# gh2o/CS184-Raytracer

Measured on NVIDIA B200. Metric: Mrays/s (primary+shadow+secondary), higher is better.
Workload: dtype f64

## Files before the change

cs184-raytracer_b200/csrc/rt_device.cuh:

```cuda
#pragma once
#include <cuda_runtime.h>
#include <stdint.h>

#include "rt_b200.h"

namespace rt {

struct d3 {
    double x, y, z;
};

__device__ __forceinline__ d3 mk3(double x, double y, double z) { d3 r; r.x = x; r.y = y; r.z = z; return r; }
__device__ __forceinline__ d3 operator+(d3 a, d3 b) { return mk3(a.x + b.x, a.y + b.y, a.z + b.z); }
__device__ __forceinline__ d3 operator-(d3 a, d3 b) { return mk3(a.x - b.x, a.y - b.y, a.z - b.z); }
__device__ __forceinline__ d3 operator-(d3 a) { return mk3(-a.x, -a.y, -a.z); }
__device__ __forceinline__ d3 operator*(double s, d3 a) { return mk3(s * a.x, s * a.y, s * a.z); }
__device__ __forceinline__ d3 vdiv(d3 a, double s) { return mk3(a.x / s, a.y / s, a.z / s); }

__device__ __forceinline__ double sum4(double a, double b, double c, double d) { return (a + c) + (b + d); }
__device__ __forceinline__ double dot4(d3 a, d3 b) { return sum4(a.x * b.x, a.y * b.y, a.z * b.z, 0.0); }
__device__ __forceinline__ double norm4(d3 a) { return sqrt(dot4(a, a)); }
__device__ __forceinline__ d3 ray_normalize(d3 a) { return vdiv(a, norm4(a)); }
__device__ __forceinline__ d3 inplace_normalize(d3 a) { return (1.0 / norm4(a)) * a; }

__device__ __forceinline__ d3 xf_point(const double* __restrict__ m, d3 v) {
    return mk3(((m[0] * v.x + m[1] * v.y) + m[2] * v.z) + m[3] * 1.0,
               ((m[4] * v.x + m[5] * v.y) + m[6] * v.z) + m[7] * 1.0,
               ((m[8] * v.x + m[9] * v.y) + m[10] * v.z) + m[11] * 1.0);
}
__device__ __forceinline__ d3 xf_dir(const double* __restrict__ m, d3 v) {
    return mk3(((m[0] * v.x + m[1] * v.y) + m[2] * v.z) + m[3] * 0.0,
               ((m[4] * v.x + m[5] * v.y) + m[6] * v.z) + m[7] * 0.0,
               ((m[8] * v.x + m[9] * v.y) + m[10] * v.z) + m[11] * 0.0);
}
__device__ __forceinline__ d3 xf_normal(const double* __restrict__ inv, d3 n) {
    return mk3(sum4(inv[0] * n.x, inv[4] * n.y, inv[8] * n.z, 0.0),
               sum4(inv[1] * n.x, inv[5] * n.y, inv[9] * n.z, 0.0),
               sum4(inv[2] * n.x, inv[6] * n.y, inv[10] * n.z, 0.0));
}

__device__ __forceinline__ double det3(d3 c0, d3 c1, d3 c2) {
    double h012 = c0.x * (c1.y * c2.z - c2.y * c1.z);
    double h102 = c1.x * (c0.y * c2.z - c2.y * c0.z);
    double h201 = c2.x * (c0.y * c1.z - c1.y * c0.z);
    return h012 - h102 + h201;
}

struct alignas(16) DGeom {
    double inv[12];
    double fwd[12];
    double det;
    double center[3];
    double radius2;
    double bbmin[3];
    double bbmax[3];
    int type;
    int mat;
    int first_face;
    int num_faces;
    int use_bbox;
    int pad_[3];
};

struct alignas(16) DMat {
    double ka[3], kd[3], ks[3], kr[3];
    double sp, ior;
    int has_kt;
    int has_kr;
    int pad_[2];
};

struct alignas(16) DLight {
    double v[3];
    double color[3];
    double falloff;
    int type;
    int pad_;
};

struct DCamera {
    double eye[3], ll[3], lr[3], ul[3], ur[3];
};

#define RT_FACE_D2 5

struct alignas(128) BvhNode {
    float4 lox, loy, loz;
    int4 ref;
    float4 hix, hiy, hiz;
    int4 pad_;
};
#define BVH_EMPTY_LO 1e30f
#define BVH_EMPTY_HI (-1e30f)
#define BVH_DONE ((int)0x80000000)

#define PRIM_KIND_SHIFT 29
#define PRIM_FACE 0
#define PRIM_SPHERE 1
#define PRIM_TRI 2
#define PRIM_INDEX_MASK ((1 << PRIM_KIND_SHIFT) - 1)

struct DScene {
    DCamera cam;
    const DGeom* geoms;
    const DMat* mats;
    const DLight* slights;
    const DLight* alights;
    const double2* face_pts;
    const double2* face_nrm;
    const BvhNode* nodes;
    const int* flat;
    const int* all_prims;
    const float4* sph_bound;
    int num_geoms;
    int num_slights;
    int num_alights;
    int num_flat;
    int num_all;
    int num_bvh_prims;
    int single_leaf;
    int shadow_mode;
    float origin_limit;
};

struct Best {
    int geom;
    int face;
    double dobj;
    double wd;
    d3 P, N;
};

struct ObjRay {
    int geom;
    int box_ok;
    d3 o, d, nd;
    double dn;
};

struct WorkCounters {
    unsigned long long nodes, tris, spheres;
};

__device__ __forceinline__ bool bbox_plane(const double* oo, const double* dd, int axis, int bn, const double* __restrict__ bbmin,
                                           const double* __restrict__ bbmax) {
    const double mag = dd[axis];
    if (mag == 0.0) return false;
    const double t = ((bn ? bbmax[axis] : bbmin[axis]) - oo[axis]) / mag;
    if (t < 0) return false;
    bool ok = true;
#pragma unroll
    for (int a2 = 0; a2 < 3; a2++) {
        if (a2 == axis) continue;
        const double ip = oo[a2] + t * dd[a2];
        if (ip < bbmin[a2] || ip > bbmax[a2]) ok = false;
    }
    return ok;
}
__device__ __forceinline__ bool mesh_bbox(d3 o, d3 d, const double* __restrict__ bbmin,
                                          const double* __restrict__ bbmax) {
    const double oo[3] = {o.x, o.y, o.z}, dd[3] = {d.x, d.y, d.z};
    {
        float best = 3.0e38f;
        int baxis = 0, bbn = 0;
#pragma unroll
        for (int axis = 0; axis < 3; axis++) {
            const float df = (float)dd[axis];
            if (df == 0.f) continue;
            const int bn = df > 0.f ? 1 : 0;
            const float tf = ((float)(bn ? bbmax[axis] : bbmin[axis]) - (float)oo[axis]) / df;
            if (tf >= 0.f && tf < best) { best = tf; baxis = axis; bbn = bn; }
        }
        if (best < 3.0e38f) {
            bool hit;
            if (baxis == 0) hit = bbox_plane(oo, dd, 0, bbn, bbmin, bbmax);
            else if (baxis == 1) hit = bbox_plane(oo, dd, 1, bbn, bbmin, bbmax);
            else hit = bbox_plane(oo, dd, 2, bbn, bbmin, bbmax);
            if (hit) return true;
        }
    }
#pragma unroll
    for (int axis = 0; axis < 3; axis++) {
#pragma unroll
        for (int bn = 0; bn < 2; bn++)
            if (bbox_plane(oo, dd, axis, bn, bbmin, bbmax)) return true;
    }
    return false;
}

__device__ __forceinline__ void load_objray(const DScene& S, int gi, d3 o, d3 d, ObjRay& R) {
    const DGeom* g = S.geoms + gi;
    R.geom = gi;
    R.o = xf_point(g->inv, o);
    R.d = ray_normalize(xf_dir(g->inv, d));
    R.nd = -R.d;
    R.dn = sqrt(R.d.x * R.d.x + (R.d.y * R.d.y + R.d.z * R.d.z));
    R.box_ok = 1;
    if (g->type == RT_GEOM_MESH && g->use_bbox) R.box_ok = mesh_bbox(R.o, R.d, g->bbmin, g->bbmax) ? 1 : 0;
}

__device__ __forceinline__ bool beats(const Best& best, int gi, int f, double dobj, double wd) {
    if (best.geom < 0) return true;
    if (gi == best.geom) return dobj < best.dobj || (dobj == best.dobj && f < best.face);
    return wd < best.wd || (wd == best.wd && gi < best.geom);
}

__device__ __forceinline__ void to_world(const DGeom* g, d3 Pobj, d3 Nobj, d3 o, d3& P, d3& N, double& wd) {
    P = xf_point(g->fwd, Pobj);
    N = xf_normal(g->inv, Nobj);
    if (g->det < 0) N = -N;
    wd = norm4(P - o);
}

template <bool ANYHIT>
__device__ __forceinline__ bool test_sphere(const DScene& S, int gi, d3 o, d3 d, bool reverse, double limit,
                                            Best& best) {
    const DGeom* g = S.geoms + gi;
    d3 oo = xf_point(g->inv, o);
    d3 dd = ray_normalize(xf_dir(g->inv, d));
    d3 c = mk3(g->center[0], g->center[1], g->center[2]);
    d3 ocd = oo - c;
    double a = dot4(dd, dd);
    double b = 2 * dot4(dd, ocd);
    double cc = dot4(ocd, ocd) - g->radius2;
    double disc = b * b - 4 * a * cc;
    if (disc < 0) return false;
    double res = reverse ? (-b + sqrt(disc)) / (2 * a) : (-b - sqrt(disc)) / (2 * a);
    if (res < 0) return false;
    d3 Pobj = oo + res * dd;
    d3 Nobj = Pobj - c;
    d3 P, N;
    double wd;
    to_world(g, Pobj, Nobj, o, P, N, wd);
    if (ANYHIT) return wd <= limit;
    if (beats(best, gi, 0, 0.0, wd)) {
        best.geom = gi; best.face = 0; best.dobj = 0.0; best.wd = wd; best.P = P; best.N = N;
    }
    return false;
}

template <bool ANYHIT>
__device__ __forceinline__ bool test_face(const DScene& S, int gi, int gface, int lface, const ObjRay& R, d3 o,
                                          bool reverse, double limit, Best& best) {
    const double2* __restrict__ fp = S.face_pts + (size_t)gface * RT_FACE_D2;
    double2 q0 = __ldg(fp + 0), q1 = __ldg(fp + 1), q2 = __ldg(fp + 2), q3 = __ldg(fp + 3), q4 = __ldg(fp + 4);
    d3 p0 = mk3(q0.x, q0.y, q1.x), va = mk3(q1.y, q2.x, q2.y), vb = mk3(q3.x, q3.y, q4.x);
    d3 rhs = R.o - p0;
    double dlower = det3(va, vb, R.nd);
    if (dlower == 0) return false;
    double a = det3(rhs, vb, R.nd) / dlower;
    if (a < 0 || a > 1) return false;
    double b = det3(va, rhs, R.nd) / dlower;
    if (b < 0 || a + b > 1) return false;
    double t = det3(va, vb, rhs) / dlower;
    if (t < 0) return false;
    double dobj = t * R.dn;
    if (!ANYHIT && best.geom == gi && (dobj > best.dobj || (dobj == best.dobj && lface > best.face))) return false;
    const double2* __restrict__ fn = S.face_nrm + (size_t)gface * RT_FACE_D2;
    double2 m0 = __ldg(fn + 0), m1 = __ldg(fn + 1), m2 = __ldg(fn + 2), m3 = __ldg(fn + 3), m4 = __ldg(fn + 4);
    d3 n0 = mk3(m0.x, m0.y, m1.x), n1 = mk3(m1.y, m2.x, m2.y), n2 = mk3(m3.x, m3.y, m4.x);
    double w0 = 1.0 - a - b;
    d3 tn = (w0 * n0 + a * n1) + b * n2;
    bool front = dot4(tn, R.d) < 0;
    if ((!front) != reverse) return false;
    d3 Pobj = p0 + (a * va + b * vb);
    d3 P, N;
    double wd;
    to_world(S.geoms + gi, Pobj, tn, o, P, N, wd);
    if (ANYHIT) return wd <= limit;
    if (beats(best, gi, lface, dobj, wd)) {
        best.geom = gi; best.face = lface; best.dobj = dobj; best.wd = wd; best.P = P; best.N = N;
    }
    return false;
}

__device__ __forceinline__ bool sphere_certainly_missed(float4 bs, d3 o, d3 d) {
    float ocx = bs.x - (float)o.x, ocy = bs.y - (float)o.y, ocz = bs.z - (float)o.z;
    float dx = (float)d.x, dy = (float)d.y, dz = (float)d.z;
    float c2 = ocx * ocx + ocy * ocy + ocz * ocz;
    float b = ocx * dx + ocy * dy + ocz * dz;
    float r = bs.w * 1.001f;
    float r2 = r * r + 1e-4f * c2 + 1e-30f;
    if (c2 - b * b > r2) return true;
    return c2 > r2 && b < -(r + 1e-3f * sqrtf(c2));
}

template <bool ANYHIT, bool COUNT>
__device__ __forceinline__ bool test_prim(const DScene& S, int code, d3 o, d3 d, bool reverse, double limit,
                                          ObjRay& R, Best& best, WorkCounters& wc) {
    const int kind = code >> PRIM_KIND_SHIFT, idx = code & PRIM_INDEX_MASK;
    if (kind == PRIM_SPHERE) {
        if (sphere_certainly_missed(__ldg(S.sph_bound + idx), o, d)) return false;
        if (COUNT) wc.spheres++;
        return test_sphere<ANYHIT>(S, idx, o, d, reverse, limit, best);
    }
    if (kind == PRIM_TRI) {
        const DGeom* g = S.geoms + idx;
        if (R.geom != idx) load_objray(S, idx, o, d, R);
        if (COUNT) wc.tris += 2;
        if (test_face<ANYHIT>(S, idx, g->first_face, 0, R, o, reverse, limit, best)) return true;
        return test_face<ANYHIT>(S, idx, g->first_face + 1, 1, R, o, reverse, limit, best);
    }
    double2 q4 = __ldg(S.face_pts + (size_t)idx * RT_FACE_D2 + 4);
    int gi = __double2loint(q4.y), lf = __double2hiint(q4.y);
    if (R.geom != gi) load_objray(S, gi, o, d, R);
    if (!R.box_ok) return false;
    if (COUNT) wc.tris++;
    return test_face<ANYHIT>(S, gi, idx, lf, R, o, reverse, limit, best);
}

struct FRay {
    float ix, iy, iz;
    float bx, by, bz;
    unsigned nx, ny, nz;
};
__device__ __forceinline__ FRay make_fray(d3 o, d3 d) {
    FRay r;
    float ox = (float)o.x, oy = (float)o.y, oz = (float)o.z;
    float dx = (float)d.x, dy = (float)d.y, dz = (float)d.z;
    const float tiny = 1e-30f;
    if (fabsf(dx) < tiny) dx = copysignf(tiny, dx);
    if (fabsf(dy) < tiny) dy = copysignf(tiny, dy);
    if (fabsf(dz) < tiny) dz = copysignf(tiny, dz);
    r.ix = 1.0f / dx; r.iy = 1.0f / dy; r.iz = 1.0f / dz;
    r.bx = -ox * r.ix; r.by = -oy * r.iy; r.bz = -oz * r.iz;
    r.nx = r.ix < 0.f ? 64u : 0u;
    r.ny = r.iy < 0.f ? 80u : 16u;
    r.nz = r.iz < 0.f ? 96u : 32u;
    asm volatile("" : "+r"(r.nx), "+r"(r.ny), "+r"(r.nz));
    return r;
}
struct Slab4 {
    float tn[4];
    bool hit[4];
};
__device__ __forceinline__ void slab1(const FRay& r, float nx, float ny, float nz, float fx, float fy, float fz,
                                      float tlimit, float& tn, bool& hit) {
    const float tnx = __fmaf_rn(nx, r.ix, r.bx), tny = __fmaf_rn(ny, r.iy, r.by), tnz = __fmaf_rn(nz, r.iz, r.bz);
    const float tfx = __fmaf_rn(fx, r.ix, r.bx), tfy = __fmaf_rn(fy, r.iy, r.by), tfz = __fmaf_rn(fz, r.iz, r.bz);
    tn = fmaxf(fmaxf(tnx, tny), fmaxf(tnz, 0.f));
    const float tf = fminf(fminf(tfx, tfy), fminf(tfz, tlimit));
    hit = tn <= tf;
}

#define RT_STACK 96
#ifndef RT_ANYHIT_UNSORTED
#define RT_ANYHIT_UNSORTED 1
#endif
#ifndef RT_SH_STACK
#define RT_SH_STACK 12
#endif
#ifndef RT_BLOCK
#define RT_BLOCK 64
#endif

__device__ __forceinline__ float prune_limit(double x) {
    if (!(x < 3.0e38)) return __int_as_float(0x7f800000);
    return __double2float_ru(x) * 1.00001f + 1e-30f;
}

#define RT_SH_ENTRY(ANYHIT) ((ANYHIT) ? 4 : 8)
#define RT_SH_STRIDE(ANYHIT) (RT_BLOCK * RT_SH_ENTRY(ANYHIT))
#define RT_SH_STACK_BYTES(ANYHIT) ((RT_SH_STACK > 0 ? RT_SH_STACK : 1) * RT_SH_STRIDE(ANYHIT))

template <bool ANYHIT>
__device__ __forceinline__ unsigned stack_base(const void* smem) {
    unsigned b = (unsigned)__cvta_generic_to_shared(smem) + threadIdx.x * RT_SH_ENTRY(ANYHIT);
    asm volatile("" : "+r"(b));
    return b;
}

template <bool ANYHIT>
struct StackSpill {
    int ref[RT_STACK];
    float t[ANYHIT ? 1 : RT_STACK];
};
template <bool ANYHIT>
struct Stack {
    unsigned base, top;
    StackSpill<ANYHIT>& sp;
    __device__ __forceinline__ Stack(unsigned shbase, StackSpill<ANYHIT>& spill) : base(shbase), top(shbase), sp(spill) {}
    __device__ __forceinline__ unsigned lim() const { return base + RT_SH_STACK * RT_SH_STRIDE(ANYHIT); }
    __device__ __forceinline__ static void sts(unsigned a, int ref, float t) {
        if (ANYHIT) asm volatile("st.shared.b32 [%0], %1;" ::"r"(a), "r"(ref));
        else asm volatile("st.shared.v2.b32 [%0], {%1, %2};" ::"r"(a), "r"(ref), "r"(__float_as_int(t)));
    }
    __device__ __forceinline__ bool roomy(int n) const { return top + n * RT_SH_STRIDE(ANYHIT) <= lim(); }
    __device__ __forceinline__ void push_fast(bool on, int ref, float t) {
        if (on) sts(top, ref, t);
        top += on ? RT_SH_STRIDE(ANYHIT) : 0;
    }
    __device__ __forceinline__ void push(int ref, float t) {
        if (top < lim()) {
            sts(top, ref, t);
        } else {
            const unsigned k = (top - lim()) / RT_SH_STRIDE(ANYHIT);
            if (k >= RT_STACK) return;
            sp.ref[k] = ref;
            if (!ANYHIT) sp.t[k] = t;
        }
        top += RT_SH_STRIDE(ANYHIT);
    }
    __device__ __forceinline__ int pop(float tlim) {
        while (top != base) {
            top -= RT_SH_STRIDE(ANYHIT);
            int ref, tb = 0;
            if (top < lim()) {
                if (ANYHIT) asm volatile("ld.shared.b32 %0, [%1];" : "=r"(ref) : "r"(top));
                else asm volatile("ld.shared.v2.b32 {%0, %1}, [%2];" : "=r"(ref), "=r"(tb) : "r"(top));
            } else {
                const unsigned k = (top - lim()) / RT_SH_STRIDE(ANYHIT);
                ref = sp.ref[k];
                if (!ANYHIT) tb = __float_as_int(sp.t[k]);
            }
            if (ANYHIT || __int_as_float(tb) <= tlim) return ref;
        }
        return BVH_DONE;
    }
};

__device__ __forceinline__ const float4* flip64(const float4* p) {
    return reinterpret_cast<const float4*>(reinterpret_cast<unsigned long long>(p) ^ 64ull);
}

template <bool ANYHIT, bool COUNT>
__device__ __forceinline__ void descend(const DScene& S, const FRay& fr, float tlim, int& cur, Stack<ANYHIT>& st,
                                        WorkCounters& wc) {
    while (cur >= 0) {
        const char* const nb = reinterpret_cast<const char*>(S.nodes);
        const unsigned off = (unsigned)cur * (unsigned)sizeof(BvhNode);
        const float4* pnx = reinterpret_cast<const float4*>(nb + (off + fr.nx));
        const float4* pny = reinterpret_cast<const float4*>(nb + (off + fr.ny));
        const float4* pnz = reinterpret_cast<const float4*>(nb + (off + fr.nz));
        const float4 nx = __ldg(pnx), ny = __ldg(pny), nz = __ldg(pnz);
        const float4 fx = __ldg(flip64(pnx)), fy = __ldg(flip64(pny)), fz = __ldg(flip64(pnz));
        const int4 ref = __ldg(reinterpret_cast<const int4*>(nb + off + 48));
        if (COUNT) wc.nodes += 4;
        float t0, t1, t2, t3;
        bool h0, h1, h2, h3;
        slab1(fr, nx.x, ny.x, nz.x, fx.x, fy.x, fz.x, tlim, t0, h0);
        slab1(fr, nx.y, ny.y, nz.y, fx.y, fy.y, fz.y, tlim, t1, h1);
        slab1(fr, nx.z, ny.z, nz.z, fx.z, fy.z, fz.z, tlim, t2, h2);
        slab1(fr, nx.w, ny.w, nz.w, fx.w, fy.w, fz.w, tlim, t3, h3);
        if (ANYHIT && RT_ANYHIT_UNSORTED) {
            int next = h3 ? ref.w : BVH_DONE;
            if (st.roomy(3)) {
                bool q;
                q = h2 && next != BVH_DONE; st.push_fast(q, next, 0.f); next = h2 ? ref.z : next;
                q = h1 && next != BVH_DONE; st.push_fast(q, next, 0.f); next = h1 ? ref.y : next;
                q = h0 && next != BVH_DONE; st.push_fast(q, next, 0.f); next = h0 ? ref.x : next;
            } else {
                if (h2) { if (next != BVH_DONE) st.push(next, 0.f); next = ref.z; }
                if (h1) { if (next != BVH_DONE) st.push(next, 0.f); next = ref.y; }
                if (h0) { if (next != BVH_DONE) st.push(next, 0.f); next = ref.x; }
            }
            cur = next != BVH_DONE ? next : st.pop(tlim);
            continue;
        }
        const unsigned MISS = 0x7f800000u;
        const unsigned k0 = h0 ? ((__float_as_uint(t0) & ~3u) | 0u) : MISS, k1 = h1 ? ((__float_as_uint(t1) & ~3u) | 1u) : MISS;
        const unsigned k2 = h2 ? ((__float_as_uint(t2) & ~3u) | 2u) : MISS, k3 = h3 ? ((__float_as_uint(t3) & ~3u) | 3u) : MISS;
        const unsigned kmin = min(min(k0, k1), min(k2, k3));
        if (st.roomy(3)) {
            st.push_fast(h3 && k3 != kmin, ref.w, t3);
            st.push_fast(h2 && k2 != kmin, ref.z, t2);
            st.push_fast(h1 && k1 != kmin, ref.y, t1);
            st.push_fast(h0 && k0 != kmin, ref.x, t0);
        } else {
            if (h3 && k3 != kmin) st.push(ref.w, t3);
            if (h2 && k2 != kmin) st.push(ref.z, t2);
            if (h1 && k1 != kmin) st.push(ref.y, t1);
            if (h0 && k0 != kmin) st.push(ref.x, t0);
        }
        if (kmin < MISS) {
            const unsigned i = kmin & 3u;
            cur = i == 0 ? ref.x : (i == 1 ? ref.y : (i == 2 ? ref.z : ref.w));
        } else {
            cur = st.pop(tlim);
        }
    }
}

template <bool ANYHIT, bool BRUTE, bool COUNT, bool FARCHECK = false>
__device__ __forceinline__ bool cast_ray(const DScene& S, d3 o, d3 d, bool reverse, double limit, Best& best,
                                         WorkCounters& wc, unsigned shbase) {
    best.geom = -1; best.face = -1; best.dobj = 0.0; best.wd = 0.0;
    ObjRay R;
    R.geom = -1; R.box_ok = 1;
    const bool far_origin = FARCHECK && !BRUTE && fmax(fabs(o.x), fmax(fabs(o.y), fabs(o.z))) > (double)S.origin_limit;
    if (BRUTE || far_origin) {
        for (int i = 0; i < S.num_all; i++)
            if (test_prim<ANYHIT, COUNT>(S, __ldg(S.all_prims + i), o, d, reverse, limit, R, best, wc)) return true;
        return false;
    }
    for (int i = 0; i < S.num_flat; i++)
        if (test_prim<ANYHIT, COUNT>(S, __ldg(S.flat + i), o, d, reverse, limit, R, best, wc)) return true;
    if (S.num_bvh_prims == 0) return false;
    if (S.num_bvh_prims == 1)
        return test_prim<ANYHIT, COUNT>(S, S.single_leaf, o, d, reverse, limit, R, best, wc);

    const FRay fr = make_fray(o, d);
    float tlim = ANYHIT ? prune_limit(limit) : __int_as_float(0x7f800000);
    StackSpill<ANYHIT> spill;
    Stack<ANYHIT> st(shbase, spill);
    int cur = 0;
    while (true) {
        descend<ANYHIT, COUNT>(S, fr, tlim, cur, st, wc);
        if (cur == BVH_DONE) break;
        if (test_prim<ANYHIT, COUNT>(S, ~cur, o, d, reverse, limit, R, best, wc)) return true;
        if (!ANYHIT && best.geom >= 0) tlim = prune_limit(best.wd);
        cur = st.pop(tlim);
        if (cur == BVH_DONE) break;
    }
    return false;
}

}
```

cs184-raytracer_b200/csrc/rt_kernels.cuh:

```cuda
#pragma once
#include "rt_device.cuh"

namespace rt {

#ifndef RT_BLOCK
#define RT_BLOCK 64
#endif
#ifndef RT_SHADOW_MINBLOCKS
#define RT_SHADOW_MINBLOCKS 16
#endif
#ifndef RT_SHADOW_TILE
#define RT_SHADOW_TILE 4096
#endif
#ifndef RT_TRACE_MINBLOCKS
#define RT_TRACE_MINBLOCKS 16
#endif

struct RayQ {
    double* f;
    int* pixel;
    int* meta;
    size_t cap;
    __device__ __forceinline__ double& fld(int k, size_t i) const { return f[(size_t)k * cap + i]; }
};
// ... 31 lines not shown
    int x = (w % (RT_TILE_W / 8)) * 8 + (l & 7), y = (w / (RT_TILE_W / 8)) * 4 + (l >> 3);
    px = tx * RT_TILE_W + x;
    py = ty * RT_TILE_H + y;
    return px < F.width && py < F.height;
}

__device__ __forceinline__ unsigned warp_append(bool flag, unsigned long long* counter) {
    unsigned m = __ballot_sync(0xffffffffu, flag);
    unsigned base = 0;
    if (m) {
        int lane = threadIdx.x & 31, leader = __ffs(m) - 1;
        if (lane == leader) base = (unsigned)atomicAdd(counter, (unsigned long long)__popc(m));
        base = __shfl_sync(0xffffffffu, base, leader);
        base += __popc(m & ((1u << lane) - 1u));
    }
    return base;
}

template <bool COUNT>
__device__ __forceinline__ void flush_work(const WorkCounters& wc, unsigned long long* ctr ) {
    if (!COUNT) return;
    unsigned long long a = wc.nodes, b = wc.tris, c = wc.spheres;
    for (int o = 16; o > 0; o >>= 1) {
        a += __shfl_down_sync(0xffffffffu, a, o);
        b += __shfl_down_sync(0xffffffffu, b, o);
        c += __shfl_down_sync(0xffffffffu, c, o);
    }
    if ((threadIdx.x & 31) == 0) {
        atomicAdd(ctr + 0, a);
        atomicAdd(ctr + 1, b);
        atomicAdd(ctr + 2, c);
    }
}

struct PrimaryRays {
    FrameInfo F;
    long long first_slot;
    int sub;
    int depth;
};
__device__ __forceinline__ int primary_ray(const DScene& S, const PrimaryRays& pr, int i, d3& E, d3& d, double& w) {
    const int ss = pr.sub * pr.sub;
    const long long slot = pr.first_slot + (pr.sub > 1 ? i / ss : i);
    int px, py;
    if (!slot_to_pixel(pr.F, slot, px, py)) return -1;
    double rowFrac = (py + 0.5) / pr.F.height, colFrac = (px + 0.5) / pr.F.width;
    w = 1.0;
    if (pr.sub > 1) {
        const int k = i % ss, si = k % pr.sub, sj = k / pr.sub;
        rowFrac = (py + (sj + 0.5) / pr.sub) / pr.F.height;
        colFrac = (px + (si + 0.5) / pr.sub) / pr.F.width;
        w = 1.0 / ss;
    }
    const DCamera& c = S.cam;
    d3 LR = mk3(c.lr[0], c.lr[1], c.lr[2]), UR = mk3(c.ur[0], c.ur[1], c.ur[2]);
    d3 LL = mk3(c.ll[0], c.ll[1], c.ll[2]), UL = mk3(c.ul[0], c.ul[1], c.ul[2]);
    E = mk3(c.eye[0], c.eye[1], c.eye[2]);
    d3 right = rowFrac * LR + (1.0 - rowFrac) * UR;
    d3 left = rowFrac * LL + (1.0 - rowFrac) * UL;
    d3 ip = colFrac * right + (1.0 - colFrac) * left;
    d3 raw = ip - E;
    const bool ok = !(raw.x == 0 && raw.y == 0 && raw.z == 0);
    d = ok ? ray_normalize(raw) : raw;
    return ok ? (int)slot : -1;
}

__global__ void __launch_bounds__(RT_BLOCK) k_raygen(DScene S, PrimaryRays pr, int n, RayQ q) {
    int i = blockIdx.x * blockDim.x + threadIdx.x;
    if (i >= n) return;
    d3 E = mk3(0, 0, 0), d = mk3(0, 0, 1);
    double w = 1.0;
    const int slot = primary_ray(S, pr, i, E, d, w);
    q.fld(0, i) = E.x; q.fld(1, i) = E.y; q.fld(2, i) = E.z;
    q.fld(3, i) = d.x; q.fld(4, i) = d.y; q.fld(5, i) = d.z;
    q.fld(6, i) = w; q.fld(7, i) = w; q.fld(8, i) = w;
    q.pixel[i] = slot;
    q.meta[i] = pr.depth;
}

template <bool BRUTE, bool COUNT, bool PRIMARY>
__global__ void __launch_bounds__(RT_BLOCK, RT_TRACE_MINBLOCKS) k_trace(DScene S, RayQ q, size_t off, int n, size_t nfront, HitQ h,
                                                     unsigned long long* ctr, int* ids_geom, int* ids_face, PrimaryRays pr) {
    __shared__ __align__(16) unsigned char sm_stack[RT_SH_STACK_BYTES(false)];
    int t = blockIdx.x * blockDim.x + threadIdx.x;
    const size_t g = off + (size_t)t;
    const size_t i = PRIMARY ? 0 : (g < nfront ? g : q.cap - 1 - (g - nfront));
    bool active = t < n;
    Best best;
    best.geom = -1;
    WorkCounters wc = {0, 0, 0};
    d3 o = mk3(0, 0, 0), d = mk3(0, 0, 1);
    double w0 = 1.0;
    int meta = 0, pixel = -1;
    if (PRIMARY) {
        if (active) pixel = primary_ray(S, pr, t, o, d, w0);
        meta = pr.depth;
    } else {
        pixel = active ? q.pixel[i] : -1;
    }
    active = active && pixel >= 0;
    if (active) {
        if (!PRIMARY) {
            o = mk3(q.fld(0, i), q.fld(1, i), q.fld(2, i));
            d = mk3(q.fld(3, i), q.fld(4, i), q.fld(5, i));
            meta = q.meta[i];
        }
        cast_ray<false, BRUTE, COUNT>(S, o, d, (meta >> RT_META_INSIDE_SHIFT) & 1, 0.0, best, wc, stack_base<false>(sm_stack));
        if (ids_geom) { ids_geom[pixel] = best.geom; ids_face[pixel] = best.face; }
    }
    bool hit = active && best.geom >= 0;
    unsigned slot = warp_append(hit, ctr + CTR_HITS);
    if (hit) {
        h.fld(0, slot) = best.P.x; h.fld(1, slot) = best.P.y; h.fld(2, slot) = best.P.z;
        h.fld(3, slot) = best.N.x; h.fld(4, slot) = best.N.y; h.fld(5, slot) = best.N.z;
        h.fld(6, slot) = d.x; h.fld(7, slot) = d.y; h.fld(8, slot) = d.z;
        if (PRIMARY) { h.fld(9, slot) = w0; h.fld(10, slot) = w0; h.fld(11, slot) = w0; }
        else { h.fld(9, slot) = q.fld(6, i); h.fld(10, slot) = q.fld(7, i); h.fld(11, slot) = q.fld(8, i); }
        h.fld(12, slot) = best.wd;
        h.pixel[slot] = pixel;
        h.geom[slot] = best.geom;
        h.meta[slot] = meta;
    }
    flush_work<COUNT>(wc, ctr + CTR_NODES);
}

struct SortGrid {
    float lo[3];
    float scale;
    int bits;
};
__device__ __forceinline__ uint32_t spread_bits3(uint32_t v) {
    v = (v * 0x00010001u) & 0xFF0000FFu;
    v = (v * 0x00000101u) & 0x0F00F00Fu;
    v = (v * 0x00000011u) & 0xC30C30C3u;
    v = (v * 0x00000005u) & 0x49249249u;
    return v;
}
__global__ void k_hit_keys(HitQ h, const unsigned long long* __restrict__ lc, SortGrid g, uint32_t* __restrict__ keys,
                           int* __restrict__ vals) {
    unsigned j = blockIdx.x * blockDim.x + threadIdx.x;
    if (j >= (unsigned)lc[CTR_HITS]) return;
    const float p[3] = {(float)h.fld(0, j), (float)h.fld(1, j), (float)h.fld(2, j)};
    uint32_t q[3];
    for (int a = 0; a < 3; a++) {
        float u = (p[a] - g.lo[a]) * g.scale;
        q[a] = (uint32_t)min(max((int)u, 0), 1023);
    }
    const uint32_t m = (spread_bits3(q[0]) << 2) | (spread_bits3(q[1]) << 1) | spread_bits3(q[2]);
    keys[j] = g.bits < 30 ? m >> (30 - g.bits) : m;
    vals[j] = (int)j;
}
__global__ void __launch_bounds__(RT_BLOCK) k_shade_io(HitQ h, const unsigned long long* ctr, double* fb,
                                                        unsigned long long* maxbits) {
    unsigned j = blockIdx.x * blockDim.x + threadIdx.x;
    double v = 0.0;
    if (j < (unsigned)ctr[CTR_HITS]) {
        double dist = h.fld(12, j);
        v = 1.0 / (dist * dist);
        size_t p = (size_t)h.pixel[j] * 3;
        fb[p] = v; fb[p + 1] = v; fb[p + 2] = v;
    }
    unsigned long long b = (unsigned long long)__double_as_longlong(v);
    for (int o = 16; o > 0; o >>= 1) {
        unsigned long long x = __shfl_down_sync(0xffffffffu, b, o);
        b = x > b ? x : b;
    }
    if ((threadIdx.x & 31) == 0 && b) atomicMax(maxbits, b);
}

__global__ void k_divide(double* fb, size_t n, const unsigned long long* maxbits) {
    size_t i = (size_t)blockIdx.x * blockDim.x + threadIdx.x;
    if (i >= n) return;
    fb[i] = fb[i] / __longlong_as_double((long long)*maxbits);
}

#ifndef RT_SHADE_BLOCK
#define RT_SHADE_BLOCK 256
#endif
__global__ void __launch_bounds__(RT_SHADE_BLOCK) k_shade(DScene S, HitQ src, HitQ h, const int* __restrict__ order,
                                                     unsigned long long* ctr, RayQ next, double* fb) {
    unsigned j = blockIdx.x * blockDim.x + threadIdx.x;
    bool active = j < (unsigned)ctr[CTR_HITS];
    bool want_t = false, want_r = false;
    d3 P = mk3(0, 0, 0), Td = P, Rd = P;
    double W[3] = {0, 0, 0}, kr[3] = {0, 0, 0};
    int pixel = 0, depth = 0, inside = 0;
    unsigned degenerate = 0;
    if (active) {
        const unsigned s = order ? (unsigned)order[j] : j;
        P = mk3(src.fld(0, s), src.fld(1, s), src.fld(2, s));
        d3 N = mk3(src.fld(3, s), src.fld(4, s), src.fld(5, s));
        d3 V = mk3(src.fld(6, s), src.fld(7, s), src.fld(8, s));
        W[0] = src.fld(9, s); W[1] = src.fld(10, s); W[2] = src.fld(11, s);
        pixel = src.pixel[s];
        int meta = src.meta[s];
        const int geom = src.geom[s];
        depth = meta & RT_META_DEPTH_MASK;
// ... 57 lines not shown
        next.pixel[sr] = pixel;
        next.meta[sr] = (depth - 1) | (inside << RT_META_INSIDE_SHIFT);
    }
    if (degenerate) atomicAdd(ctr + CTR_DEGENERATE, (unsigned long long)degenerate);
}

__device__ __forceinline__ double pow_shading(double x, double y) {
    if (y >= 1.0 && y <= 1024.0 && y == floor(y)) {
        unsigned n = (unsigned)y;
        double r = 1.0, b = x;
        while (true) {
            if (n & 1u) r *= b;
            n >>= 1;
            if (!n) break;
            b *= b;
        }
        return r;
    }
    return pow(x, y);
}

template <bool BRUTE, bool COUNT>
__global__ void __launch_bounds__(RT_BLOCK, RT_SHADOW_MINBLOCKS) k_shadow(DScene S, HitQ h, unsigned long long* ctr, double* fb) {
    __shared__ __align__(16) unsigned char sm_stack[RT_SH_STACK_BYTES(true)];
    unsigned long long t = (unsigned long long)blockIdx.x * blockDim.x + threadIdx.x;
    const unsigned nsl = (unsigned)S.num_slights;
    WorkCounters wc = {0, 0, 0};
    const unsigned long long nhits = ctr[CTR_HITS];
    if (t < nhits * nsl) {
        unsigned li, j;
        if (S.shadow_mode & 1) {
#if RT_SHADOW_TILE > 0
            unsigned long long tile;
            if (nhits * nsl <= 0xffffffffull) tile = (unsigned)t / (RT_SHADOW_TILE * nsl);
            else tile = t / ((unsigned long long)RT_SHADOW_TILE * nsl);
            const unsigned long long first = tile * RT_SHADOW_TILE;
            const unsigned w = (unsigned)min((unsigned long long)RT_SHADOW_TILE, nhits - first);
            const unsigned r = (unsigned)(t - tile * RT_SHADOW_TILE * nsl);
            li = r / w; j = (unsigned)first + r % w;
#else
            li = (unsigned)(t / nhits); j = (unsigned)(t % nhits);
#endif
        } else { j = (unsigned)(t / nsl); li = (unsigned)(t % nsl); }
        const DLight* l = S.slights + li;
        d3 P = mk3(h.fld(0, j), h.fld(1, j), h.fld(2, j));
        d3 N = mk3(h.fld(3, j), h.fld(4, j), h.fld(5, j));
        d3 lv = mk3(l->v[0], l->v[1], l->v[2]);
        const bool point = l->type == RT_LIGHT_POINT;
        d3 toL = point ? lv - P : -lv;
        if (toL.x == 0 && toL.y == 0 && toL.z == 0) {
            atomicAdd(ctr + CTR_DEGENERATE, 1ull);
        } else {
            d3 L = ray_normalize(toL);
            double ndl = dot4(N, L);
            bool lrev = ndl < 0;
            const double INF = __longlong_as_double(0x7ff0000000000000ll);
            double dL = point ? norm4(toL) : INF;
            int inside = (h.meta[j] >> RT_META_INSIDE_SHIFT) & 1;
            const DMat* m = S.mats + S.geoms[h.geom[j]].mat;
            d3 V = mk3(h.fld(6, j), h.fld(7, j), h.fld(8, j));
            double att[3];
            if (point) {
                const double fo = l->falloff;
                double f = fo == 0.0 ? 1.0 : (fo == 1.0 ? 1.0 / dL : (fo == 2.0 ? 1.0 / (dL * dL) : pow(dL, -fo)));
                for (int k = 0; k < 3; k++) att[k] = f * l->color[k];
            } else {
                for (int k = 0; k < 3; k++) att[k] = l->color[k];
            }
            double di = ndl < 0.0 ? 0.0 : ndl;
            d3 R = (2 * ndl) * N - L;
            double mvr = -dot4(V, R);
            const double sp_ = m->sp;
            double si = (mvr < 0.0 && sp_ > 0.0) ? 0.0 : pow_shading(mvr < 0.0 ? 0.0 : mvr, sp_);
            double c[3];
            bool any = false;
            for (int k = 0; k < 3; k++) {
                double w = h.fld(9 + k, j);
                c[k] = w * (di * att[k] * m->kd[k]) + w * (si * att[k] * m->ks[k]);
                any = any || !(c[k] == 0.0);
            }
            if (COUNT && !any) atomicAdd(ctr + CTR_S_CULLED, 1ull);
            if (any) {
                Best best;
                bool occluded = cast_ray<true, BRUTE, COUNT>(S, P, L, lrev != (inside != 0), dL, best, wc, stack_base<true>(sm_stack));
                if (!occluded) {
                    int pixel = h.pixel[j];
                    for (int k = 0; k < 3; k++) atomicAdd(fb + (size_t)pixel * 3 + k, c[k]);
                }
            }
        }
    }
    flush_work<COUNT>(wc, ctr + CTR_S_NODES);
}

__device__ __forceinline__ unsigned char quantize(double v) {
    v = (1.0 < v) ? 1.0 : v;
    v = (v < 0.0) ? 0.0 : v;
    if (v != v) v = 0.0;
    return (unsigned char)(int)(v * 255.0);
}
template <bool QUANT>
__global__ void k_resolve(FrameInfo F, const double* __restrict__ fb, long long nslots, int full, void* out) {
    long long slot = (long long)blockIdx.x * blockDim.x + threadIdx.x;
    if (slot >= nslots) return;
    int px, py;
    bool inside = slot_to_pixel(F, slot, px, py);
    size_t dst;
    if (full) {
        if (!inside) return;
        dst = ((size_t)py * F.width + px) * 3;
    } else {
        dst = (size_t)slot * 3;
    }
    for (int k = 0; k < 3; k++) {
        double v = inside ? fb[(size_t)slot * 3 + k] : 0.0;
        if (QUANT) ((unsigned char*)out)[dst + k] = quantize(v);
        else ((double*)out)[dst + k] = v;
    }
}

#if RT_TILE_W == 32
__global__ void __launch_bounds__(256) k_resolve_rgb8_rows(FrameInfo F, const double* __restrict__ fb, long long nslots,
                                                            unsigned char* __restrict__ out) {
    __shared__ __align__(16) unsigned char rows[8][96];
    const long long slot0 = (long long)blockIdx.x * 256;
    const long long slot = slot0 + threadIdx.x;
    int px, py;
    const bool inside = slot < nslots && slot_to_pixel(F, slot, px, py);
    {
        const int j = threadIdx.x, w = j >> 5, l = j & 31;
        const int x = (w & 3) * 8 + (l & 7), y = (w >> 2) * 4 + (l >> 3);
        for (int k = 0; k < 3; k++) rows[y][3 * x + k] = inside ? quantize(fb[(size_t)slot * 3 + k]) : 0;
    }
    __syncthreads();
    int px0, py0;
    if (slot0 >= nslots) return;
    slot_to_pixel(F, slot0, px0, py0);
    if (threadIdx.x < 192) {
        const int r = threadIdx.x / 24, wd = threadIdx.x % 24;
        const int y = py0 + r;
        if (y < F.height) {
            const size_t base = ((size_t)y * F.width + px0) * 3;
            if (px0 + 32 <= F.width && (base & 3) == 0) {
                *reinterpret_cast<unsigned*>(out + base + 4 * wd) = *reinterpret_cast<const unsigned*>(&rows[r][4 * wd]);
            } else {
                const int nb = 3 * min(32, F.width - px0);
                for (int bidx = 4 * wd; bidx < 4 * wd + 4; bidx++)
                    if (bidx < nb) out[base + bidx] = rows[r][bidx];
            }
        }
    }
}
#endif

template <typename T>
__global__ void k_unpack(int width, int height, int tiles_x, int world, long long max_tiles,
                         const int* __restrict__ rank_row_start , int tiles_y,
                         const T* __restrict__ packed, T* __restrict__ frame) {
    long long i = (long long)blockIdx.x * blockDim.x + threadIdx.x;
    if (i >= (long long)width * height) return;
    int px = (int)(i % width), py = (int)(i / width);
    int tx = px / RT_TILE_W, ty = py / RT_TILE_H;
    int rank = (tx + ty) % world;
    int first_tx = ((rank - ty) % world + world) % world;
    long long lt = rank_row_start[rank * (tiles_y + 1) + ty] + (tx - first_tx) / world;
    int x = px % RT_TILE_W, y = py % RT_TILE_H;
    int w = (y / 4) * (RT_TILE_W / 8) + (x / 8), l = (y % 4) * 8 + (x % 8);
    long long slot = ((long long)rank * max_tiles + lt) * RT_TILE_PIXELS + w * 32 + l;
    for (int k = 0; k < 3; k++) frame[i * 3 + k] = packed[slot * 3 + k];
}

template <bool BRUTE>
__global__ void __launch_bounds__(RT_BLOCK) k_query(DScene S, long long n, const double* __restrict__ org,
                                                     const double* __restrict__ dir,
                                                     const unsigned char* __restrict__ reverse, int* geom, int* face,
                                                     double* dist, double* point, double* normal) {
    __shared__ __align__(16) unsigned char sm_stack[RT_SH_STACK_BYTES(false)];
    long long i = (long long)blockIdx.x * blockDim.x + threadIdx.x;
    if (i >= n) return;
    d3 o = mk3(org[3 * i], org[3 * i + 1], org[3 * i + 2]);
    d3 raw = mk3(dir[3 * i], dir[3 * i + 1], dir[3 * i + 2]);
    Best best;
    best.geom = -1; best.face = -1; best.wd = 0; best.P = mk3(0, 0, 0); best.N = mk3(0, 0, 0);
    WorkCounters wc = {0, 0, 0};
    if (raw.x == 0 && raw.y == 0 && raw.z == 0) {
        best.geom = -2;
    } else {
        cast_ray<false, BRUTE, false, true>(S, o, ray_normalize(raw), reverse ? reverse[i] != 0 : false, 0.0, best, wc, stack_base<false>(sm_stack));
    }
    bool hit = best.geom >= 0;
    if (geom) geom[i] = best.geom;
    if (face) face[i] = hit ? best.face : -1;
    if (dist) dist[i] = hit ? best.wd : 0.0;
    if (point) { point[3 * i] = hit ? best.P.x : 0; point[3 * i + 1] = hit ? best.P.y : 0; point[3 * i + 2] = hit ? best.P.z : 0; }
    if (normal) { normal[3 * i] = hit ? best.N.x : 0; normal[3 * i + 1] = hit ? best.N.y : 0; normal[3 * i + 2] = hit ? best.N.z : 0; }
}

__global__ void k_gather_probe(const float4* __restrict__ data, unsigned long long nrec, int loads, float* sink) {
    unsigned long long t = (unsigned long long)blockIdx.x * blockDim.x + threadIdx.x;
    unsigned long long x = t * 0x9E3779B97F4A7C15ull + 0x1234567ull;
    float acc = 0.f;
    for (int i = 0; i < loads; i++) {
        x ^= x >> 30; x *= 0xBF58476D1CE4E5B9ull; x ^= x >> 27; x *= 0x94D049BB133111EBull; x ^= x >> 31;
        unsigned long long r = x % nrec;
        float4 a = __ldg(data + 2 * r), b = __ldg(data + 2 * r + 1);
        acc += a.x + b.w;
    }
    if (acc == 123.456f) *sink = acc;
}

__global__ void __launch_bounds__(RT_BLOCK, RT_SHADOW_MINBLOCKS) k_node_walk(const BvhNode* __restrict__ nodes, int visits,
                                                                              int group, float* sink) {
    const unsigned t = blockIdx.x * blockDim.x + threadIdx.x;
    const unsigned path = t / (unsigned)group;
    unsigned long long x = (unsigned long long)path * 0x9E3779B97F4A7C15ull + 0x1234567ull;
    x ^= x >> 30; x *= 0xBF58476D1CE4E5B9ull; x ^= x >> 27;
    const unsigned nx = (x & 1) ? 64u : 0u, ny = (x & 2) ? 80u : 16u, nz = (x & 4) ? 96u : 32u;
    float acc = 0.f;
    int cur = 0;
    const char* const nb = reinterpret_cast<const char*>(nodes);
    for (int v = 0; v < visits; v++) {
        const unsigned off = (unsigned)cur * (unsigned)sizeof(BvhNode);
        const float4* pnx = reinterpret_cast<const float4*>(nb + (off + nx));
        const float4* pny = reinterpret_cast<const float4*>(nb + (off + ny));
        const float4* pnz = reinterpret_cast<const float4*>(nb + (off + nz));
        const float4 a = __ldg(pnx), b = __ldg(pny), c = __ldg(pnz);
        const float4 d = __ldg(flip64(pnx)), e = __ldg(flip64(pny)), f = __ldg(flip64(pnz));
        const int4 ref = __ldg(reinterpret_cast<const int4*>(nb + off + 48));
        acc += a.x + b.y + c.z + d.w + e.x + f.y;
        x = x * 6364136223846793005ull + 1442695040888963407ull;
        const unsigned r = (unsigned)(x >> 33);
        const int cand[4] = {ref.x, ref.y, ref.z, ref.w};
        int next = 0;
#pragma unroll
        for (int k = 3; k >= 0; k--) {
            const int cc = cand[(r + k) & 3];
            next = cc >= 0 ? cc : next;
        }
        cur = next;
    }
    if (acc == 123.456f) *sink = acc;
}

struct FaceOwner {
    int geom, first, count;
    int all_off;
    int bvh_off;
};

__global__ void k_pack_faces(long long nf, const double* __restrict__ pts, const double* __restrict__ nrm,
                             const FaceOwner* __restrict__ owners, int nowners, double2* __restrict__ out_p,
                             double2* __restrict__ out_n, int* __restrict__ all_prims, int* __restrict__ bvh_prims) {
    long long f = (long long)blockIdx.x * blockDim.x + threadIdx.x;
    if (f >= nf) return;
    int lo = 0, hi = nowners;
    while (lo < hi) {
        int mid = (lo + hi) >> 1;
        if (owners[mid].first <= (int)f) lo = mid + 1;
        else hi = mid;
    }
    int fgeom = 0, flocal = 0;
    if (lo > 0) {
        const FaceOwner o = owners[lo - 1];
        if ((int)f - o.first < o.count) {
            fgeom = o.geom;
            flocal = (int)f - o.first;
            if (o.all_off >= 0) {
                const int code = (PRIM_FACE << PRIM_KIND_SHIFT) | (int)f;
                all_prims[o.all_off + flocal] = code;
                bvh_prims[o.bvh_off + flocal] = code;
            }
        }
    }
    const double* p = pts + 9 * f;
    const double* n = nrm + 9 * f;
    d3 p0 = mk3(p[0], p[1], p[2]), p1 = mk3(p[3], p[4], p[5]), p2 = mk3(p[6], p[7], p[8]);
    d3 va = p1 - p0, vb = p2 - p0;
    double aux = __hiloint2double(flocal, fgeom);
// ... 21 lines not shown
```

Before: 4885.

## Spill ray/objray state to shared memory and recompute hit surface after traversal

Drops the hit point and normal from the per-thread best-hit record and recomputes them once after traversal by re-intersecting the winning primitive. In the trace and query kernels, the world and object-space ray (origin, direction, norm) now live in a per-thread shared-memory slot read through inline PTX, and the shadow kernel keeps them in a register array. It also removes the cached negated direction and skips faces early when the cached object-ray bbox test failed. The aim is to cut register pressure in the hot traversal loop and raise occupancy, at the cost of extra shared loads per primitive test and a second intersection per hit.

```diff
diff --git a/cs184-raytracer_b200/csrc/rt_device.cuh b/cs184-raytracer_b200/csrc/rt_device.cuh
--- a/cs184-raytracer_b200/csrc/rt_device.cuh
+++ b/cs184-raytracer_b200/csrc/rt_device.cuh
@@ -5,6 +5,10 @@
 #include "rt_b200.h"
 
 namespace rt {
+
+#ifndef RT_BLOCK
+#define RT_BLOCK 64
+#endif
 
 struct d3 {
     double x, y, z;
@@ -128,13 +132,12 @@
     int face;
     double dobj;
     double wd;
-    d3 P, N;
 };
 
 struct ObjRay {
     int geom;
     int box_ok;
-    d3 o, d, nd;
+    d3 o, d;
     double dn;
 };
 
@@ -193,7 +196,6 @@
     R.geom = gi;
     R.o = xf_point(g->inv, o);
     R.d = ray_normalize(xf_dir(g->inv, d));
-    R.nd = -R.d;
     R.dn = sqrt(R.d.x * R.d.x + (R.d.y * R.d.y + R.d.z * R.d.z));
     R.box_ok = 1;
     if (g->type == RT_GEOM_MESH && g->use_bbox) R.box_ok = mesh_bbox(R.o, R.d, g->bbmin, g->bbmax) ? 1 : 0;
@@ -212,10 +214,7 @@
     wd = norm4(P - o);
 }
 
-template <bool ANYHIT>
-__device__ __forceinline__ bool test_sphere(const DScene& S, int gi, d3 o, d3 d, bool reverse, double limit,
-                                            Best& best) {
-    const DGeom* g = S.geoms + gi;
+__device__ __forceinline__ bool sphere_hit(const DGeom* g, d3 o, d3 d, bool reverse, d3& P, d3& N, double& wd) {
     d3 oo = xf_point(g->inv, o);
     d3 dd = ray_normalize(xf_dir(g->inv, d));
     d3 c = mk3(g->center[0], g->center[1], g->center[2]);
@@ -229,33 +228,39 @@
     if (res < 0) return false;
     d3 Pobj = oo + res * dd;
     d3 Nobj = Pobj - c;
+    to_world(g, Pobj, Nobj, o, P, N, wd);
+    return true;
+}
+
+template <bool ANYHIT>
+__device__ __forceinline__ bool test_sphere(const DScene& S, int gi, d3 o, d3 d, bool reverse, double limit,
+                                            Best& best) {
     d3 P, N;
     double wd;
-    to_world(g, Pobj, Nobj, o, P, N, wd);
+    if (!sphere_hit(S.geoms + gi, o, d, reverse, P, N, wd)) return false;
     if (ANYHIT) return wd <= limit;
     if (beats(best, gi, 0, 0.0, wd)) {
-        best.geom = gi; best.face = 0; best.dobj = 0.0; best.wd = wd; best.P = P; best.N = N;
+        best.geom = gi; best.face = 0; best.dobj = 0.0; best.wd = wd;
     }
     return false;
 }
 
-template <bool ANYHIT>
-__device__ __forceinline__ bool test_face(const DScene& S, int gi, int gface, int lface, const ObjRay& R, d3 o,
-                                          bool reverse, double limit, Best& best) {
+__device__ __forceinline__ bool face_hit(const DScene& S, int gi, int gface, int lface, const ObjRay& R, d3 o,
+                                         bool reverse, const Best& best, double& dobj, d3& P, d3& N, double& wd) {
     const double2* __restrict__ fp = S.face_pts + (size_t)gface * RT_FACE_D2;
     double2 q0 = __ldg(fp + 0), q1 = __ldg(fp + 1), q2 = __ldg(fp + 2), q3 = __ldg(fp + 3), q4 = __ldg(fp + 4);
     d3 p0 = mk3(q0.x, q0.y, q1.x), va = mk3(q1.y, q2.x, q2.y), vb = mk3(q3.x, q3.y, q4.x);
     d3 rhs = R.o - p0;
-    double dlower = det3(va, vb, R.nd);
+    double dlower = det3(va, vb, -R.d);
     if (dlower == 0) return false;
-    double a = det3(rhs, vb, R.nd) / dlower;
+    double a = det3(rhs, vb, -R.d) / dlower;
     if (a < 0 || a > 1) return false;
-    double b = det3(va, rhs, R.nd) / dlower;
+    double b = det3(va, rhs, -R.d) / dlower;
     if (b < 0 || a + b > 1) return false;
     double t = det3(va, vb, rhs) / dlower;
     if (t < 0) return false;
-    double dobj = t * R.dn;
-    if (!ANYHIT && best.geom == gi && (dobj > best.dobj || (dobj == best.dobj && lface > best.face))) return false;
+    dobj = t * R.dn;
+    if (best.geom == gi && (dobj > best.dobj || (dobj == best.dobj && lface > best.face))) return false;
     const double2* __restrict__ fn = S.face_nrm + (size_t)gface * RT_FACE_D2;
     double2 m0 = __ldg(fn + 0), m1 = __ldg(fn + 1), m2 = __ldg(fn + 2), m3 = __ldg(fn + 3), m4 = __ldg(fn + 4);
     d3 n0 = mk3(m0.x, m0.y, m1.x), n1 = mk3(m1.y, m2.x, m2.y), n2 = mk3(m3.x, m3.y, m4.x);
@@ -264,12 +269,21 @@
     bool front = dot4(tn, R.d) < 0;
     if ((!front) != reverse) return false;
     d3 Pobj = p0 + (a * va + b * vb);
+    to_world(S.geoms + gi, Pobj, tn, o, P, N, wd);
+    return true;
+}
+
+template <bool ANYHIT>
+__device__ __forceinline__ bool test_face(const DScene& S, int gi, int gface, int lface, const ObjRay& R, d3 o,
+                                          bool reverse, double limit, Best& best) {
+    Best none;
+    none.geom = -1;
+    double dobj, wd;
     d3 P, N;
-    double wd;
-    to_world(S.geoms + gi, Pobj, tn, o, P, N, wd);
+    if (!face_hit(S, gi, gface, lface, R, o, reverse, ANYHIT ? none : best, dobj, P, N, wd)) return false;
     if (ANYHIT) return wd <= limit;
     if (beats(best, gi, lface, dobj, wd)) {
-        best.geom = gi; best.face = lface; best.dobj = dobj; best.wd = wd; best.P = P; best.N = N;
+        best.geom = gi; best.face = lface; best.dobj = dobj; best.wd = wd;
     }
     return false;
 }
@@ -285,28 +299,84 @@
     return c2 > r2 && b < -(r + 1e-3f * sqrtf(c2));
 }
 
-template <bool ANYHIT, bool COUNT>
-__device__ __forceinline__ bool test_prim(const DScene& S, int code, d3 o, d3 d, bool reverse, double limit,
-                                          ObjRay& R, Best& best, WorkCounters& wc) {
+#define RT_LEAF_O 0
+#define RT_LEAF_D 3
+#define RT_LEAF_RO 6
+#define RT_LEAF_RD 9
+#define RT_LEAF_RDN 12
+#define RT_LEAF_WORDS 13
+#define RT_LEAF_BYTES (RT_LEAF_WORDS * RT_BLOCK * 8)
+
+struct LeafShared {
+    unsigned a;
+    __device__ __forceinline__ explicit LeafShared(const void* smem) {
+        a = (unsigned)__cvta_generic_to_shared(smem) + threadIdx.x * 8;
+        asm volatile("" : "+r"(a));
+    }
+    __device__ __forceinline__ double ld(int k) const {
+        double v;
+        asm volatile("ld.shared.f64 %0, [%1];" : "=d"(v) : "r"(a + k * RT_BLOCK * 8));
+        return v;
+    }
+    __device__ __forceinline__ void st(int k, double v) const {
+        asm volatile("st.shared.f64 [%0], %1;" ::"r"(a + k * RT_BLOCK * 8), "d"(v));
+    }
+};
+struct LeafRegs {
+    double w[RT_LEAF_WORDS];
+    __device__ __forceinline__ double ld(int k) const { return w[k]; }
+    __device__ __forceinline__ void st(int k, double v) { w[k] = v; }
+};
+template <class Leaf>
+__device__ __forceinline__ d3 leaf_ld3(const Leaf& leaf, int k) {
+    return mk3(leaf.ld(k), leaf.ld(k + 1), leaf.ld(k + 2));
+}
+template <class Leaf>
+__device__ __forceinline__ void leaf_st3(Leaf& leaf, int k, d3 v) {
+    leaf.st(k, v.x); leaf.st(k + 1, v.y); leaf.st(k + 2, v.z);
+}
+
+template <class Leaf>
+__device__ __forceinline__ ObjRay leaf_objray(const DScene& S, int gi, Leaf& leaf, int& cached, int& box_ok) {
+    ObjRay R;
+    if (cached != gi) {
+        load_objray(S, gi, leaf_ld3(leaf, RT_LEAF_O), leaf_ld3(leaf, RT_LEAF_D), R);
+        leaf_st3(leaf, RT_LEAF_RO, R.o); leaf_st3(leaf, RT_LEAF_RD, R.d); leaf.st(RT_LEAF_RDN, R.dn);
+        cached = gi;
+        box_ok = R.box_ok;
+    } else {
+        R.geom = gi;
+        R.box_ok = box_ok;
+        R.o = leaf_ld3(leaf, RT_LEAF_RO); R.d = leaf_ld3(leaf, RT_LEAF_RD); R.dn = leaf.ld(RT_LEAF_RDN);
+    }
+    return R;
+}
+
+template <bool ANYHIT, bool COUNT, class Leaf>
+__device__ __forceinline__ bool test_prim(const DScene& S, int code, Leaf& leaf, bool reverse, double limit,
+                                          int& cached, int& box_ok, Best& best, WorkCounters& wc) {
     const int kind = code >> PRIM_KIND_SHIFT, idx = code & PRIM_INDEX_MASK;
     if (kind == PRIM_SPHERE) {
+        const d3 o = leaf_ld3(leaf, RT_LEAF_O), d = leaf_ld3(leaf, RT_LEAF_D);
         if (sphere_certainly_missed(__ldg(S.sph_bound + idx), o, d)) return false;
         if (COUNT) wc.spheres++;
         return test_sphere<ANYHIT>(S, idx, o, d, reverse, limit, best);
     }
     if (kind == PRIM_TRI) {
         const DGeom* g = S.geoms + idx;
-        if (R.geom != idx) load_objray(S, idx, o, d, R);
+        const ObjRay R = leaf_objray(S, idx, leaf, cached, box_ok);
+        const d3 o = leaf_ld3(leaf, RT_LEAF_O);
         if (COUNT) wc.tris += 2;
         if (test_face<ANYHIT>(S, idx, g->first_face, 0, R, o, reverse, limit, best)) return true;
         return test_face<ANYHIT>(S, idx, g->first_face + 1, 1, R, o, reverse, limit, best);
     }
     double2 q4 = __ldg(S.face_pts + (size_t)idx * RT_FACE_D2 + 4);
     int gi = __double2loint(q4.y), lf = __double2hiint(q4.y);
-    if (R.geom != gi) load_objray(S, gi, o, d, R);
+    if (cached == gi && !box_ok) return false;
+    const ObjRay R = leaf_objray(S, gi, leaf, cached, box_ok);
     if (!R.box_ok) return false;
     if (COUNT) wc.tris++;
-    return test_face<ANYHIT>(S, gi, idx, lf, R, o, reverse, limit, best);
+    return test_face<ANYHIT>(S, gi, idx, lf, R, leaf_ld3(leaf, RT_LEAF_O), reverse, limit, best);
 }
 
 struct FRay {
@@ -349,9 +419,6 @@
 #endif
 #ifndef RT_SH_STACK
 #define RT_SH_STACK 12
-#endif
-#ifndef RT_BLOCK
-#define RT_BLOCK 64
 #endif
 
 __device__ __forceinline__ float prune_limit(double x) {
@@ -481,23 +548,24 @@
     }
 }
 
-template <bool ANYHIT, bool BRUTE, bool COUNT, bool FARCHECK = false>
+template <bool ANYHIT, bool BRUTE, bool COUNT, bool FARCHECK = false, class Leaf>
 __device__ __forceinline__ bool cast_ray(const DScene& S, d3 o, d3 d, bool reverse, double limit, Best& best,
-                                         WorkCounters& wc, unsigned shbase) {
+                                         WorkCounters& wc, unsigned shbase, Leaf& leaf) {
     best.geom = -1; best.face = -1; best.dobj = 0.0; best.wd = 0.0;
-    ObjRay R;
-    R.geom = -1; R.box_ok = 1;
+    int cached = -1, box_ok = 1;
+    leaf_st3(leaf, RT_LEAF_O, o);
+    leaf_st3(leaf, RT_LEAF_D, d);
     const bool far_origin = FARCHECK && !BRUTE && fmax(fabs(o.x), fmax(fabs(o.y), fabs(o.z))) > (double)S.origin_limit;
     if (BRUTE || far_origin) {
         for (int i = 0; i < S.num_all; i++)
-            if (test_prim<ANYHIT, COUNT>(S, __ldg(S.all_prims + i), o, d, reverse, limit, R, best, wc)) return true;
+            if (test_prim<ANYHIT, COUNT>(S, __ldg(S.all_prims + i), leaf, reverse, limit, cached, box_ok, best, wc)) return true;
         return false;
     }
     for (int i = 0; i < S.num_flat; i++)
-        if (test_prim<ANYHIT, COUNT>(S, __ldg(S.flat + i), o, d, reverse, limit, R, best, wc)) return true;
+        if (test_prim<ANYHIT, COUNT>(S, __ldg(S.flat + i), leaf, reverse, limit, cached, box_ok, best, wc)) return true;
     if (S.num_bvh_prims == 0) return false;
     if (S.num_bvh_prims == 1)
-        return test_prim<ANYHIT, COUNT>(S, S.single_leaf, o, d, reverse, limit, R, best, wc);
+        return test_prim<ANYHIT, COUNT>(S, S.single_leaf, leaf, reverse, limit, cached, box_ok, best, wc);
 
     const FRay fr = make_fray(o, d);
     float tlim = ANYHIT ? prune_limit(limit) : __int_as_float(0x7f800000);
@@ -507,7 +575,7 @@
     while (true) {
         descend<ANYHIT, COUNT>(S, fr, tlim, cur, st, wc);
         if (cur == BVH_DONE) break;
-        if (test_prim<ANYHIT, COUNT>(S, ~cur, o, d, reverse, limit, R, best, wc)) return true;
+        if (test_prim<ANYHIT, COUNT>(S, ~cur, leaf, reverse, limit, cached, box_ok, best, wc)) return true;
         if (!ANYHIT && best.geom >= 0) tlim = prune_limit(best.wd);
         cur = st.pop(tlim);
         if (cur == BVH_DONE) break;
@@ -515,4 +583,19 @@
     return false;
 }
 
-}
+__device__ __forceinline__ void hit_surface(const DScene& S, const Best& best, d3 o, d3 d, bool reverse, d3& P, d3& N) {
+    const DGeom* g = S.geoms + best.geom;
+    double wd;
+    if (g->type == RT_GEOM_SPHERE) {
+        sphere_hit(g, o, d, reverse, P, N, wd);
+        return;
+    }
+    ObjRay R;
+    load_objray(S, best.geom, o, d, R);
+    Best none;
+    none.geom = -1;
+    double dobj;
+    face_hit(S, best.geom, g->first_face + best.face, best.face, R, o, reverse, none, dobj, P, N, wd);
+}
+
+}
diff --git a/cs184-raytracer_b200/csrc/rt_kernels.cuh b/cs184-raytracer_b200/csrc/rt_kernels.cuh
--- a/cs184-raytracer_b200/csrc/rt_kernels.cuh
+++ b/cs184-raytracer_b200/csrc/rt_kernels.cuh
@@ -137,6 +137,8 @@
 __global__ void __launch_bounds__(RT_BLOCK, RT_TRACE_MINBLOCKS) k_trace(DScene S, RayQ q, size_t off, int n, size_t nfront, HitQ h,
                                                      unsigned long long* ctr, int* ids_geom, int* ids_face, PrimaryRays pr) {
     __shared__ __align__(16) unsigned char sm_stack[RT_SH_STACK_BYTES(false)];
+    __shared__ __align__(16) unsigned char sm_leaf[RT_LEAF_BYTES];
+    LeafShared leaf(sm_leaf);
     int t = blockIdx.x * blockDim.x + threadIdx.x;
     const size_t g = off + (size_t)t;
     const size_t i = PRIMARY ? 0 : (g < nfront ? g : q.cap - 1 - (g - nfront));
@@ -160,14 +162,18 @@
             d = mk3(q.fld(3, i), q.fld(4, i), q.fld(5, i));
             meta = q.meta[i];
         }
-        cast_ray<false, BRUTE, COUNT>(S, o, d, (meta >> RT_META_INSIDE_SHIFT) & 1, 0.0, best, wc, stack_base<false>(sm_stack));
+        cast_ray<false, BRUTE, COUNT>(S, o, d, (meta >> RT_META_INSIDE_SHIFT) & 1, 0.0, best, wc, stack_base<false>(sm_stack), leaf);
         if (ids_geom) { ids_geom[pixel] = best.geom; ids_face[pixel] = best.face; }
     }
     bool hit = active && best.geom >= 0;
     unsigned slot = warp_append(hit, ctr + CTR_HITS);
     if (hit) {
-        h.fld(0, slot) = best.P.x; h.fld(1, slot) = best.P.y; h.fld(2, slot) = best.P.z;
-        h.fld(3, slot) = best.N.x; h.fld(4, slot) = best.N.y; h.fld(5, slot) = best.N.z;
+        o = leaf_ld3(leaf, RT_LEAF_O);
+        d = leaf_ld3(leaf, RT_LEAF_D);
+        d3 P, N;
+        hit_surface(S, best, o, d, (meta >> RT_META_INSIDE_SHIFT) & 1, P, N);
+        h.fld(0, slot) = P.x; h.fld(1, slot) = P.y; h.fld(2, slot) = P.z;
+        h.fld(3, slot) = N.x; h.fld(4, slot) = N.y; h.fld(5, slot) = N.z;
         h.fld(6, slot) = d.x; h.fld(7, slot) = d.y; h.fld(8, slot) = d.z;
         if (PRIMARY) { h.fld(9, slot) = w0; h.fld(10, slot) = w0; h.fld(11, slot) = w0; }
         else { h.fld(9, slot) = q.fld(6, i); h.fld(10, slot) = q.fld(7, i); h.fld(11, slot) = q.fld(8, i); }
@@ -391,7 +397,8 @@
             if (COUNT && !any) atomicAdd(ctr + CTR_S_CULLED, 1ull);
             if (any) {
                 Best best;
-                bool occluded = cast_ray<true, BRUTE, COUNT>(S, P, L, lrev != (inside != 0), dL, best, wc, stack_base<true>(sm_stack));
+                LeafRegs leaf;
+                bool occluded = cast_ray<true, BRUTE, COUNT>(S, P, L, lrev != (inside != 0), dL, best, wc, stack_base<true>(sm_stack), leaf);
                 if (!occluded) {
                     int pixel = h.pixel[j];
                     for (int k = 0; k < 3; k++) atomicAdd(fb + (size_t)pixel * 3 + k, c[k]);
@@ -485,24 +492,30 @@
                                                      const unsigned char* __restrict__ reverse, int* geom, int* face,
                                                      double* dist, double* point, double* normal) {
     __shared__ __align__(16) unsigned char sm_stack[RT_SH_STACK_BYTES(false)];
+    __shared__ __align__(16) unsigned char sm_leaf[RT_LEAF_BYTES];
     long long i = (long long)blockIdx.x * blockDim.x + threadIdx.x;
     if (i >= n) return;
     d3 o = mk3(org[3 * i], org[3 * i + 1], org[3 * i + 2]);
     d3 raw = mk3(dir[3 * i], dir[3 * i + 1], dir[3 * i + 2]);
     Best best;
-    best.geom = -1; best.face = -1; best.wd = 0; best.P = mk3(0, 0, 0); best.N = mk3(0, 0, 0);
+    best.geom = -1; best.face = -1; best.wd = 0;
+    d3 P = mk3(0, 0, 0), N = mk3(0, 0, 0);
     WorkCounters wc = {0, 0, 0};
     if (raw.x == 0 && raw.y == 0 && raw.z == 0) {
         best.geom = -2;
     } else {
-        cast_ray<false, BRUTE, false, true>(S, o, ray_normalize(raw), reverse ? reverse[i] != 0 : false, 0.0, best, wc, stack_base<false>(sm_stack));
+        const d3 d = ray_normalize(raw);
+        const bool rev = reverse ? reverse[i] != 0 : false;
+        LeafShared leaf(sm_leaf);
+        cast_ray<false, BRUTE, false, true>(S, o, d, rev, 0.0, best, wc, stack_base<false>(sm_stack), leaf);
+        if (best.geom >= 0) hit_surface(S, best, o, d, rev, P, N);
     }
     bool hit = best.geom >= 0;
     if (geom) geom[i] = best.geom;
     if (face) face[i] = hit ? best.face : -1;
     if (dist) dist[i] = hit ? best.wd : 0.0;
-    if (point) { point[3 * i] = hit ? best.P.x : 0; point[3 * i + 1] = hit ? best.P.y : 0; point[3 * i + 2] = hit ? best.P.z : 0; }
-    if (normal) { normal[3 * i] = hit ? best.N.x : 0; normal[3 * i + 1] = hit ? best.N.y : 0; normal[3 * i + 2] = hit ? best.N.z : 0; }
+    if (point) { point[3 * i] = P.x; point[3 * i + 1] = P.y; point[3 * i + 2] = P.z; }
+    if (normal) { normal[3 * i] = N.x; normal[3 * i + 1] = N.y; normal[3 * i + 2] = N.z; }
 }
 
 __global__ void k_gather_probe(const float4* __restrict__ data, unsigned long long nrec, int loads, float* sink) {
```

Measured after the change: 5127, median of 6. 1.05x the previous value.
